# seemapoudel58/Physics_informed_image_segmentation

Hardware: AMD Instinct MI355X
Metric: training images/sec (512x512, Stage-II RD+PF loss) (higher is better)
Workload: dtype fp32 (fp16x3 split MFMA, power-of-two block scales; direct + Winograd convs); 1 GPU; C2: UNet(1,1,64) bs=8/GPU 512x512 Stage-II (lambda_RD=lambda_PF=1e-4, D=5, a=0.5, eps=0.05) AdamW lr=1e-5; global_batch=8, parallelism=dp1

## Files before the change

### include/pis_capi.h

```cpp
#ifndef PIS_CAPI_H
#define PIS_CAPI_H

#include <stddef.h>
#include <stdint.h>

#ifdef __cplusplus
extern "C" {
#endif

typedef void* pis_stream_t;

#define PIS_OK 0
#define PIS_ERR_ARG (-1)
#define PIS_ERR_LAUNCH (-2)
#define PIS_ERR_WORKSPACE (-3)

#define PIS_RELU 1
#define PIS_SCALE 2
#define PIS_MASK 4
#define PIS_ACCUMULATE 8
#define PIS_WINO_PREPARED 16
#define PIS_W_UNFLIPPED 32
#define PIS_FILTER_READY 64

const char* pis_last_error(void);
int pis_version(void);

#define PIS_TUNE_IGEMM_BK 1
#define PIS_TUNE_DEBUG_NOLOAD 2
#define PIS_TUNE_CONV_HALO 3
#define PIS_TUNE_HALO_VARIANT 4
#define PIS_TUNE_WGRAD_VARIANT 5
#define PIS_TUNE_WGRAD_BLOCKS 6
#define PIS_TUNE_C1_WGRAD 7
#define PIS_TUNE_WINOGRAD 8
#define PIS_TUNE_WINO_WGRAD_BLOCKS 9
#define PIS_TUNE_WINO_TILE 10
#define PIS_TUNE_WINO_F4 11
#define PIS_TUNE_WINO_FUSED 12
#define PIS_TUNE_CONVT_GEMM 13
#define PIS_TUNE_WGRAD_X6 14
#define PIS_TUNE_WINO_GEMM_OUT 15
#define PIS_TUNE_WINO_DZ2 16
#define PIS_TUNE_WINO_VW 17
#define PIS_TUNE_LOSS_ROWS 18
#define PIS_TUNE_LOSS_ROWMUL 19
#define PIS_TUNE_SLAB_CHUNKS 20
#define PIS_TUNE_WGRAD_PAIR 21
#define PIS_TUNE_WINO_GEMM_OUT_H3 22
#define PIS_TUNE_WINO_H3_PRE 23
#define PIS_TUNE_WINO_PERSIST 24
#define PIS_TUNE_FUSED_STAGGER 25
#define PIS_TUNE_FUSED_WIDE 26
#define PIS_TUNE_FUSED_K128 27
#define PIS_TUNE_FUSED_PAIR 28
#define PIS_TUNE_DIRECT_H3 29
#define PIS_TUNE_DIRECT_WG 30
#define PIS_TUNE_WGRAD_T 31
#define PIS_TUNE_DIRECT_PIPE 32
#define PIS_TUNE_DIRECT_W8 33
#define PIS_TUNE_DIRECT_WSTRIP 34
#define PIS_TUNE_DIRECT_WBLOCKS 35
#define PIS_TUNE_HEAD_LOSS_ROWS 36
#define PIS_TUNE_DIRECT_WGRAD_ALL 37
#define PIS_TUNE_HEAD_LOSS_WIDE 38
#define PIS_TUNE_WGRAD_T_DEPTH 39
#define PIS_TUNE_DZ_VW 40
#define PIS_TUNE_GEMM_256 41
#define PIS_TUNE_LAST_WGRAD_MAIN 42
#define PIS_TUNE_DIRECT_W_VWALK 43
#define PIS_TUNE_DIRECT_WGRAD_MAIN 44
#define PIS_TUNE_GEMM_PRIO 45
#define PIS_TUNE_WINO_OUT_MPF 46
#define PIS_TUNE_WINO_F6 47
#define PIS_TUNE_WGRAD_OUT 48
#define PIS_TUNE_DIRECT_W_ROWS 49
#define PIS_TUNE_WINO_XFORM 50
#define PIS_TUNE_WINO_DGRAD_T 51
#define PIS_TUNE_PROB_VARIANT 52
#define PIS_TUNE_DIRECT_MFMA16 53
#define PIS_TUNE_EVOLVE_T 54
#define PIS_TUNE_EDT_PRUNE 55
#define PIS_TUNE_NKEYS 56
#define PIS_DEBUG_NOLOAD (1 << 16)
int pis_tune(int key, int value);
int pis_debug_gemm_nt(const float* A, const float* B, float* C, int M, int N, int K, int batch, int variant,
                      pis_stream_t stream);
int pis_debug_stream_probe(const float* a, const float* b, float* dst, int64_t n, float* partial, int grid,
                           pis_stream_t stream);

int pis_debug_band_probe(const float* a, int64_t n, int mode, float* partial, int grid, pis_stream_t stream);

int pis_arm_gemm_event(void* event);

int pis_stream_create(int priority, pis_stream_t* out);
int pis_stream_destroy(pis_stream_t stream);
int pis_stream_capture_status(pis_stream_t stream);

typedef void (*pis_launch_hook_t)(const char* kernel, int phase, pis_stream_t stream, double flop,
                                  void* user);
void pis_set_launch_hook(pis_launch_hook_t fn, void* user);

int pis_conv3x3_fwd(const float* x, int ldx, const float* w_krsc, const float* bias,
                    const float* scale, float* y, int ldy, int B, int H, int W, int Cin,
                    int Cout, int flags, pis_stream_t stream);
size_t pis_conv3x3_ex_ws(int B, int H, int W, int Cin, int Cout);
int pis_conv3x3_fwd_ex(const float* x, int ldx, const float* w_krsc, const float* bias,
                       const float* scale, float* y, int ldy, int B, int H, int W, int Cin, int Cout,
                       int flags, void* ws, size_t ws_bytes, pis_stream_t stream);
int pis_conv3x3_flip(const float* w_krsc, float* w_flip, int Cin, int Cout, pis_stream_t stream);
int pis_conv3x3_dgrad(const float* dz, int ldz, const float* w_flip, const float* mask, int ldm,
                      const float* scale, float* dx, int lddx, int B, int H, int W, int Cin,
                      int Cout, int flags, pis_stream_t stream);
int pis_conv3x3_dgrad_ex(const float* dz, int ldz, const float* w_flip, const float* mask, int ldm,
                         const float* scale, float* dx, int lddx, int B, int H, int W, int Cin,
                         int Cout, int flags, void* ws, size_t ws_bytes, pis_stream_t stream);
size_t pis_conv3x3_keep_bytes(int B, int H, int W, int Cin, int Cout);
int pis_conv3x3_fwd_keep(const float* x, int ldx, const float* w_krsc, const float* bias,
                         const float* scale, float* y, int ldy, int B, int H, int W, int Cin, int Cout,
                         int flags, void* ws, size_t ws_bytes, float* keep, pis_stream_t stream);
int pis_conv3x3_fwd_pool(const float* x, int ldx, const float* w_krsc, const float* bias, const float* scale,
                         float* y, int ldy, int B, int H, int W, int Cin, int Cout, int flags, void* ws,
                         size_t ws_bytes, float* keep, float* pool, pis_stream_t stream);
int pis_conv3x3_wgrad_keep(const float* x, int ldx, const float* dz, int ldz, float* dw_krsc, float* db,
                           int B, int H, int W, int Cin, int Cout, int flags, void* ws, size_t ws_bytes,
                           const float* keep, pis_stream_t stream);
size_t pis_conv3x3_filter_bytes(int B, int H, int W, int Cin, int Cout, int dgrad);
int pis_conv3x3_filter(const float* w, int B, int H, int W, int Cin, int Cout, int dgrad, void* out,
                       size_t out_bytes, pis_stream_t stream);
typedef struct pis_filter_job {
  const float* w;
  void* out;
  size_t out_bytes;
  int B, H, W, Cin, Cout, dgrad;
} pis_filter_job;
#define PIS_FILTER_MAX_JOBS 40
int pis_conv3x3_filter_format(int B, int H, int W, int Cin, int Cout, int dgrad);
int pis_conv3x3_filters(const pis_filter_job* jobs, int n, pis_stream_t stream);
int pis_conv3x3_dgrad_direct(int B, int H, int W, int Cin, int Cout, int ldz, size_t ws_bytes);
int pis_conv3x3_bwd_prep(const float* dz, int ldz, int B, int H, int W, int Cin, int Cout, void* ws_dgrad,
                         size_t ws_dgrad_bytes, void* ws_wgrad, size_t ws_wgrad_bytes, pis_stream_t stream);
size_t pis_conv3x3_wgrad_ws(int B, int H, int W, int Cin, int Cout);
int pis_conv3x3_wgrad(const float* x, int ldx, const float* dz, int ldz, float* dw_krsc, float* db,
                      int B, int H, int W, int Cin, int Cout, int flags, void* ws, size_t ws_bytes,
                      pis_stream_t stream);

int pis_convt2x2_fwd(const float* x, int ldx, const float* w_ijoc, const float* bias, float* y,
                     int ldy, int B, int H, int W, int Cin, int Cout, pis_stream_t stream);
int pis_convt2x2_prep(const float* w_ijoc, float* w_cijo, int Cin, int Cout, pis_stream_t stream);
int pis_convt2x2_dgrad(const float* dy, int lddy, const float* w_cijo, const float* mask, int ldm,
                       float* dx, int lddx, int B, int H, int W, int Cin, int Cout, int flags,
                       pis_stream_t stream);
size_t pis_convt2x2_wgrad_ws(int B, int H, int W, int Cin, int Cout);
int pis_convt2x2_wgrad(const float* x, int ldx, const float* dy, int lddy, float* dw_ijoc,
                       float* db, int B, int H, int W, int Cin, int Cout, int flags, void* ws,
                       size_t ws_bytes, pis_stream_t stream);

int pis_maxpool2x2_fwd(const float* x, int ldx, float* y, int B, int H, int W, int C,
                       pis_stream_t stream);
int pis_maxpool2x2_bwd(const float* x, int ldx, const float* dy, const float* dskip, int ldskip,
                       float* dx, int lddx, int B, int H, int W, int C, pis_stream_t stream);

int pis_head_fwd(const float* x, int ldx, const float* w, const float* b, float* z, float* u,
                 int64_t npix, int C, pis_stream_t stream);
size_t pis_head_bwd_ws(int64_t npix, int C);
int pis_head_bwd(const float* x, int ldx, const float* w, const float* g, const float* u, float* dx,
                 int lddx, float* dw, float* db, int64_t npix, int C, int flags, void* ws,
                 size_t ws_bytes, pis_stream_t stream);

typedef struct pis_loss_params {
  float dice_w, bce_w;
  float rd_w, pf_w;
  float smooth;
  float D, a;
  float eps;
  float thr;
  int flags;
} pis_loss_params;
#define PIS_LOSS_ALL_TERMS 1
#define PIS_LOSS_CHAIN_SIGMOID 2
#define PIS_LOSS_NO_REACTION 4
#define PIS_LOSS_NTERMS 8
size_t pis_loss_ws(int B, int H, int W);
int pis_loss_fwd(const float* p, const float* t, int B, int H, int W, const pis_loss_params* prm,
                 float* out_terms, int* counts, float* scores, void* ws, size_t ws_bytes,
                 pis_stream_t stream);
int pis_loss_bwd(const float* p, const float* t, int B, int H, int W, const pis_loss_params* prm,
                 const float* terms, const float* grad_out, float* dst, int flags,
                 pis_stream_t stream);

size_t pis_head_loss_fwd_ws(int B, int H, int W);
int pis_head_loss_fwd_ok(int B, int H, int W, int C);
int pis_head_loss_fwd(const float* x, int ldx, const float* w, const float* bias, const float* t, float* z,
                      float* u, int B, int H, int W, int C, const pis_loss_params* prm, float* out_terms,
                      int* counts, float* scores, void* ws, size_t ws_bytes, pis_stream_t stream);
size_t pis_head_loss_bwd_ws(int B, int H, int W, int C);
int pis_head_loss_bwd(const float* x, int ldx, const float* w, const float* u, const float* t,
                      float* du_out, int B, int H, int W, int C, const pis_loss_params* prm,
                      const float* terms, const float* grad_out, float* dx, int lddx, float* dw,
                      float* db, int flags, void* ws, size_t ws_bytes, pis_stream_t stream);
int pis_pde_fields(const float* u, int B, int H, int W, float D, float a, float* lap,
                   float* residual, float* gradmag2, pis_stream_t stream);
int pis_pde_fields_bwd(const float* u, const float* g_lap, const float* g_residual,
                       const float* g_gradmag2, int B, int H, int W, float D, float a, float* du,
                       pis_stream_t stream);

int pis_adamw_step(float* p, const float* g, float* m, float* v, int64_t n, double lr, double beta1,
                   double beta2, double eps, double weight_decay, double step_size, double bc2_sqrt,
                   double grad_scale, pis_stream_t stream);

#define PIS_GRADNORM_SKIP_NONFINITE 1
#define PIS_GRADNORM_NSTATS 8
size_t pis_grad_sumsq_ws(int n_seg, int64_t n_total);
int pis_grad_sumsq(const float* g, const int64_t* seg_off, const int64_t* seg_len, int n_seg,
                   double grad_scale, double max_norm ,
                   int flags , double* seg_sumsq, void* record,
                   void* stats, void* ws, size_t ws_bytes, pis_stream_t stream);
int pis_adamw_step_clipped(float* p, const float* g, float* m, float* v, int64_t n, double lr,
                           double beta1, double beta2, double eps, double weight_decay,
                           double step_size, double bc2_sqrt, double grad_scale, const void* record,
                           pis_stream_t stream);

int pis_adamw_step_ema(float* p, const float* g, float* m, float* v, float* ema, int64_t n, double lr,
                       double beta1, double beta2, double eps, double weight_decay, double step_size,
                       double bc2_sqrt, double grad_scale, double ema_weight,
                       const void* record , pis_stream_t stream);
int pis_arena_exchange(float* a, float* b, int64_t n, pis_stream_t stream);

size_t pis_colsum_ws(int64_t npix, int C);
int pis_colsum(const float* src, int ld, int64_t npix, int C, float* out, int flags, void* ws,
               size_t ws_bytes, pis_stream_t stream);

size_t pis_synth_ws(int B, int H, int W);
int pis_synth_discs(const float* discs, const int* ndisc, int max_discs, uint64_t seed,
                    const int64_t* sample_ids, float* img, float* mask, int B, int H, int W,
                    void* ws, size_t ws_bytes, pis_stream_t stream);

size_t pis_boundary_ws(int B, int H, int W);
int pis_boundary_metrics(const float* p, const float* t, int B, int H, int W, float thr, int tolerance,
// ... 58 lines not shown
```

### physics_informed_image_segmentation_amd/_hip.py

```python
from __future__ import annotations

import ctypes
import os
from ctypes import c_double, c_float, c_int, c_int64, c_size_t, c_void_p
from typing import Optional

import torch

_HERE = os.path.dirname(os.path.abspath(__file__))
LIB_PATH = os.path.join(_HERE, "_lib", "libpis.so")

PIS_RELU, PIS_SCALE, PIS_MASK, PIS_ACCUMULATE, PIS_WINO_PREPARED, PIS_W_UNFLIPPED = 1, 2, 4, 8, 16, 32
PIS_FILTER_READY = 64
PIS_LOSS_ALL_TERMS, PIS_LOSS_CHAIN_SIGMOID, PIS_LOSS_NO_REACTION = 1, 2, 4
PIS_TUNE_LAST_WGRAD_MAIN = 42
PIS_TUNE_DIRECT_MFMA16 = 53
PIS_TUNE_PROB_VARIANT = 52
PIS_TUNE_EVOLVE_T = 54
PIS_TUNE_EDT_PRUNE = 55
PIS_EVOLVE_CLAMP, PIS_EVOLVE_TILE_H, PIS_EVOLVE_TILE_W, PIS_EVOLVE_MAX_STEPS = 1, 32, 64, 65536
PIS_CACHE_IMG_U8, PIS_CACHE_IMG_F32, PIS_CACHE_MASK_BITS, PIS_CACHE_MASK_F32 = 0, 1, 0, 1
PIS_GRADNORM_SKIP_NONFINITE, PIS_GRADNORM_NSTATS = 1, 8
LOSS_NTERMS = 8
TERM_TOTAL, TERM_DICE, TERM_BCE, TERM_RD, TERM_PF, TERM_I, TERM_P, TERM_T = range(8)


class FilterJob(ctypes.Structure):
    _fields_ = [("w", c_void_p), ("out", c_void_p), ("out_bytes", c_size_t), ("B", c_int), ("H", c_int),
                ("W", c_int), ("Cin", c_int), ("Cout", c_int), ("dgrad", c_int)]


class LossParams(ctypes.Structure):
    _fields_ = [("dice_w", c_float), ("bce_w", c_float), ("rd_w", c_float), ("pf_w", c_float),
                ("smooth", c_float), ("D", c_float), ("a", c_float), ("eps", c_float),
                ("thr", c_float), ("flags", c_int)]


P, I, L, Z, Dbl = c_void_p, c_int, c_int64, c_size_t, c_double
LAUNCH_HOOK_T = ctypes.CFUNCTYPE(None, ctypes.c_char_p, c_int, c_void_p, ctypes.c_double, c_void_p)

_SIGNATURES = {
    "pis_set_launch_hook": ([LAUNCH_HOOK_T, P], None),
    "pis_arm_gemm_event": ([P], c_int),
    "pis_stream_create": ([I, ctypes.POINTER(c_void_p)], c_int),
    "pis_stream_destroy": ([P], c_int),
    "pis_stream_capture_status": ([P], c_int),
    "pis_version": ([], c_int),
    "pis_last_error": ([], ctypes.c_char_p),
    "pis_tune": ([I, I], c_int),
    "pis_debug_gemm_nt": ([P, P, P, I, I, I, I, I, P], c_int),
    "pis_debug_stream_probe": ([P, P, P, L, P, I, P], c_int),
    "pis_debug_band_probe": ([P, L, I, P, I, P], c_int),
    "pis_conv3x3_dgrad_direct": ([I, I, I, I, I, I, Z], c_int),
    "pis_conv3x3_bwd_prep": ([P, I, I, I, I, I, I, P, Z, P, Z, P], c_int),
    "pis_conv3x3_filter_bytes": ([I, I, I, I, I, I], c_size_t),
    "pis_conv3x3_filter_format": ([I, I, I, I, I, I], c_int),
    "pis_conv3x3_filter": ([P, I, I, I, I, I, I, P, Z, P], c_int),
    "pis_conv3x3_filters": ([P, I, P], c_int),
    "pis_conv3x3_fwd_pool": ([P, I, P, P, P, P, I, I, I, I, I, I, I, P, Z, P, P, P], c_int),
    "pis_conv3x3_fwd": ([P, I, P, P, P, P, I, I, I, I, I, I, I, P], c_int),
    "pis_conv3x3_flip": ([P, P, I, I, P], c_int),
    "pis_conv3x3_dgrad": ([P, I, P, P, I, P, P, I, I, I, I, I, I, I, P], c_int),
    "pis_conv3x3_ex_ws": ([I, I, I, I, I], c_size_t),
    "pis_conv3x3_fwd_ex": ([P, I, P, P, P, P, I, I, I, I, I, I, I, P, Z, P], c_int),
    "pis_conv3x3_dgrad_ex": ([P, I, P, P, I, P, P, I, I, I, I, I, I, I, P, Z, P], c_int),
    "pis_conv3x3_wgrad_ws": ([I, I, I, I, I], c_size_t),
    "pis_conv3x3_keep_bytes": ([I, I, I, I, I], c_size_t),
    "pis_conv3x3_fwd_keep": ([P, I, P, P, P, P, I, I, I, I, I, I, I, P, Z, P, P], c_int),
    "pis_conv3x3_wgrad_keep": ([P, I, P, I, P, P, I, I, I, I, I, I, P, Z, P, P], c_int),
    "pis_conv3x3_wgrad": ([P, I, P, I, P, P, I, I, I, I, I, I, P, Z, P], c_int),
    "pis_convt2x2_fwd": ([P, I, P, P, P, I, I, I, I, I, I, P], c_int),
    "pis_convt2x2_prep": ([P, P, I, I, P], c_int),
    "pis_convt2x2_dgrad": ([P, I, P, P, I, P, I, I, I, I, I, I, I, P], c_int),
    "pis_convt2x2_wgrad_ws": ([I, I, I, I, I], c_size_t),
    "pis_convt2x2_wgrad": ([P, I, P, I, P, P, I, I, I, I, I, I, P, Z, P], c_int),
    "pis_maxpool2x2_fwd": ([P, I, P, I, I, I, I, P], c_int),
    "pis_maxpool2x2_bwd": ([P, I, P, P, I, P, I, I, I, I, I, P], c_int),
    "pis_head_fwd": ([P, I, P, P, P, P, L, I, P], c_int),
    "pis_head_bwd_ws": ([L, I], c_size_t),
    "pis_head_bwd": ([P, I, P, P, P, P, I, P, P, L, I, I, P, Z, P], c_int),
    "pis_loss_ws": ([I, I, I], c_size_t),
    "pis_loss_fwd": ([P, P, I, I, I, ctypes.POINTER(LossParams), P, P, P, P, Z, P], c_int),
    "pis_loss_bwd": ([P, P, I, I, I, ctypes.POINTER(LossParams), P, P, P, I, P], c_int),
    "pis_head_loss_fwd_ws": ([I, I, I], c_size_t),
    "pis_head_loss_fwd_ok": ([I, I, I, I], c_int),
    "pis_head_loss_fwd": ([P, I, P, P, P, P, P, I, I, I, I, ctypes.POINTER(LossParams), P, P, P, P, Z, P], c_int),
    "pis_head_loss_bwd_ws": ([I, I, I, I], c_size_t),
    "pis_head_loss_bwd": ([P, I, P, P, P, P, I, I, I, I, ctypes.POINTER(LossParams), P, P, P, I, P, P, I, P, Z,
                           P], c_int),
    "pis_adamw_step": ([P, P, P, P, L, Dbl, Dbl, Dbl, Dbl, Dbl, Dbl, Dbl, Dbl, P], c_int),
    "pis_grad_sumsq_ws": ([I, L], c_size_t),
    "pis_grad_sumsq": ([P, P, P, I, Dbl, Dbl, I, P, P, P, P, Z, P], c_int),
    "pis_adamw_step_clipped": ([P, P, P, P, L, Dbl, Dbl, Dbl, Dbl, Dbl, Dbl, Dbl, Dbl, P, P], c_int),
    "pis_adamw_step_ema": ([P, P, P, P, P, L, Dbl, Dbl, Dbl, Dbl, Dbl, Dbl, Dbl, Dbl, Dbl, P, P], c_int),
    "pis_arena_exchange": ([P, P, L, P], c_int),
    "pis_colsum_ws": ([L, I], c_size_t),
    "pis_colsum": ([P, I, L, I, P, I, P, Z, P], c_int),
    "pis_pde_fields": ([P, I, I, I, c_float, c_float, P, P, P, P], c_int),
    "pis_pde_fields_bwd": ([P, P, P, P, I, I, I, c_float, c_float, P, P], c_int),
    "pis_synth_ws": ([I, I, I], c_size_t),
    "pis_synth_discs": ([P, P, I, ctypes.c_uint64, P, P, P, I, I, I, P, Z, P], c_int),
    "pis_boundary_ws": ([I, I, I], c_size_t),
    "pis_boundary_metrics": ([P, P, I, I, I, c_float, I, P, P, P, P, Z, P], c_int),
    "pis_objects_ws": ([I, I, I], c_size_t),
    "pis_object_metrics": ([P, P, I, I, I, c_float, I, I, P, P, P, P, Z, P], c_int),
    "pis_probability_ws": ([I, I, I], c_size_t),
    "pis_probability_table": ([P, P, I, I, I, P, P, P, Z, P], c_int),
    "pis_cache_batch": ([P, I, Z, P, I, Z, P, P, P, L, P, P, I, I, I, P], c_int),
    "pis_cache_batch_affine": ([P, I, Z, P, I, Z, P, P, P, L, P, P, I, I, I, P], c_int),
    "pis_tile_count": ([I, I, I, I, I, ctypes.POINTER(c_int), ctypes.POINTER(c_int)], c_int),
    "pis_tile_gather": ([P, I, Z, P, I, I, I, I, I, I, I, L, L, P, P], c_int),
    "pis_tile_blend": ([P, I, I, I, I, I, I, I, c_float, P, P, P], c_int),
    "pis_pde_evolve_ws": ([I, I, I, I], c_size_t),
    "pis_pde_evolve": ([P, P, P, P, I, I, I, c_float, c_float, c_float, c_float, c_float, I, I, c_float, P, Z, P],
                       c_int),
    "pis_pde_energies_ws": ([I, I, I], c_size_t),
    "pis_pde_energies": ([P, I, I, I, c_float, c_float, c_float, P, P, P, Z, P], c_int),
    "pis_edt_ws": ([I, I, I], c_size_t),
    "pis_edt_sq": ([P, I, I, I, P, P, Z, P], c_int),
    "pis_surface_distances_ws": ([I, I, I], c_size_t),
    "pis_surface_distances": ([P, P, I, I, I, P, P, P, Z, P], c_int),
}

_lib: Optional[ctypes.CDLL] = None


class HipError(RuntimeError):
    pass


def lib() -> ctypes.CDLL:
    global _lib
    if _lib is None:
        if not os.path.exists(LIB_PATH):
            raise HipError(f"HIP extension not built: {LIB_PATH} is missing "
                           "(run __graft_entry__.build() or `python -m physics_informed_image_segmentation_amd.build`)")
        import torch
        so = ctypes.CDLL(LIB_PATH)
        for name, (argtypes, restype) in _SIGNATURES.items():
            fn = getattr(so, name)
            fn.argtypes = argtypes
            fn.restype = restype
        _lib = so
    return _lib


def exported_symbols():
    return list(_SIGNATURES)


def ptr(t: Optional[torch.Tensor]) -> int:
    return 0 if t is None else t.data_ptr()


def stream_handle(device: Optional[torch.device] = None) -> int:
    return torch.cuda.current_stream(device).cuda_stream


# ... 108 lines not shown
```

### physics_informed_image_segmentation_amd/csrc/capi.hip

```cpp
#include <atomic>
#include <cstdarg>

#include "common.h"

namespace pis {
static thread_local char g_last_error[512] = "";

void set_error(const char* fmt, ...) {
  va_list ap;
  va_start(ap, fmt);
  vsnprintf(g_last_error, sizeof(g_last_error), fmt, ap);
  va_end(ap);
}

static std::atomic<int> g_tune[PIS_TUNE_NKEYS] = {0, 16, 0, 1, 0, 1, 512, 0, 1, 1024, 4, 1, 0, 4, 3, 1, 1, 2,
                                                   1, 1, 1, 0, 1, 0, 0, 0, 2, 1, 0, 1, 0, 1, 1, 0, 0, 512, 0, 0, 1, 2, 2, 0, 1, 1, 0, 0, 1,
                                                   0, 1, 2, 1, 1, 0, 3, 8, 3};

int tune_get(int key) { return (key > 0 && key < PIS_TUNE_NKEYS) ? g_tune[key].load() : 0; }

static std::atomic<pis_launch_hook_t> g_hook{nullptr};
static std::atomic<void*> g_hook_user{nullptr};

void launch_hook(const char* kernel, int phase, hipStream_t s, double flop) {
  const pis_launch_hook_t fn = g_hook.load(std::memory_order_relaxed);
  if (fn) fn(kernel, phase, (pis_stream_t)s, flop, g_hook_user.load(std::memory_order_relaxed));
}

static thread_local hipEvent_t g_gemm_event = nullptr;

void gemm_done(hipStream_t s) {
  if (g_gemm_event) {
    (void)hipEventRecord(g_gemm_event, s);
    g_gemm_event = nullptr;
  }
}
}

extern "C" const char* pis_last_error(void) { return pis::g_last_error; }
extern "C" int pis_version(void) { return 1; }

extern "C" int pis_arm_gemm_event(void* event) {
  const int pending = pis::g_gemm_event != nullptr;
  pis::g_gemm_event = (hipEvent_t)event;
  return pending;
}

extern "C" int pis_stream_create(int priority, pis_stream_t* out) {
  PIS_CHECK_ARG(out != nullptr, "pis_stream_create: out is NULL");
  hipStream_t s = nullptr;
  const hipError_t e = hipStreamCreateWithPriority(&s, hipStreamNonBlocking, priority);
  if (e != hipSuccess) {
    pis::set_error("pis_stream_create: %s", hipGetErrorString(e));
    return PIS_ERR_LAUNCH;
  }
  *out = (pis_stream_t)s;
  return PIS_OK;
}

extern "C" int pis_stream_destroy(pis_stream_t stream) {
  PIS_CHECK_ARG(stream != nullptr, "pis_stream_destroy: NULL stream");
  const hipError_t e = hipStreamDestroy((hipStream_t)stream);
  if (e != hipSuccess) {
    pis::set_error("pis_stream_destroy: %s", hipGetErrorString(e));
    return PIS_ERR_LAUNCH;
  }
  return PIS_OK;
}

extern "C" int pis_stream_capture_status(pis_stream_t stream) {
  hipStreamCaptureStatus st = hipStreamCaptureStatusNone;
  const hipError_t e = hipStreamIsCapturing((hipStream_t)stream, &st);
  if (e != hipSuccess) {
    pis::set_error("pis_stream_capture_status: %s", hipGetErrorString(e));
    return PIS_ERR_LAUNCH;
  }
  return (int)st;
}

extern "C" void pis_set_launch_hook(pis_launch_hook_t fn, void* user) {
  pis::g_hook_user.store(user);
  pis::g_hook.store(fn);
}

extern "C" int pis_tune(int key, int value) {
  if (key <= 0 || key >= PIS_TUNE_NKEYS) {
    pis::set_error("pis_tune: unknown key %d", key);
    return PIS_ERR_ARG;
  }
  if (key == PIS_TUNE_IGEMM_BK && value >= 0 && value != 16 && value != 32) {
    pis::set_error("pis_tune: igemm K-step must be 16 or 32");
    return PIS_ERR_ARG;
  }
  if (key == PIS_TUNE_EVOLVE_T && value >= 0 && value != 1 && value != 2 && value != 4 && value != 8) {
    pis::set_error("pis_tune: the temporal block of pis_pde_evolve must be 1, 2, 4 or 8");
    return PIS_ERR_ARG;
  }
  if (key == PIS_TUNE_EDT_PRUNE && value >= 0 && value != 0 && value != 1 && value != 3) {
    pis::set_error("pis_tune: the pruning of the distance transform's row pass must be 0, 1 or 3");
    return PIS_ERR_ARG;
// ... 6 lines not shown
```

### physics_informed_image_segmentation_amd/csrc/wgrad.hip

```cpp
#include "conv3x3_plan.h"

namespace pis {

enum BMode { B_PLAIN = 0, B_CONV3 = 1, B_CONV3_C1 = 2 };

struct WgradArgs {
  const float* a; int lda; int a_up2; int Ca;
  const float* b; int ldb; int b_mode; int Cb;
  int B, H, W;
  int P;
  int Mp, Np;
  int pix_per_split;
  float* part;
  float* part_bias;
  int64_t bs_a, bs_b, bs_part, split_stride;
  int pair;
  int bias_xi;
  int dbg;
};

template <int BM, int BN, int BKP>
__global__ __launch_bounds__(256) void wgrad_f32_kernel(WgradArgs g) {
  const Remap2 rm = xcd_remap2();
  if (rm.batch) {
// ... 1049 lines not shown
#pragma unroll
          for (int a = 0; a < 2; ++a)
#pragma unroll
            for (int b = 0; b < 2; ++b) acc[a][b] = (acc[a][b] * fa) * fb;
        }
        ua = sa;
        ub = sb;
      }
    }
#pragma unroll
    for (int ks = 0; ks < 2; ++ks) {
      if (ks) {
#pragma unroll
        for (int pl = 0; pl < 2; ++pl)
#pragma unroll
          for (int a = 0; a < 2; ++a) {
            af[pl][a] = frag(buf + pl * WT_PLANE, 1, 64 * wm + 32 * a);
            bf[pl][a] = frag(buf + (2 + pl) * WT_PLANE, 1, 64 * wn + 32 * a);
          }
      }
#pragma unroll
      for (int a = 0; a < 2; ++a)
#pragma unroll
        for (int b = 0; b < 2; ++b) {
          acc[a][b] = __builtin_amdgcn_mfma_f32_32x32x16_f16(af[1][a], bf[0][b], acc[a][b], 0, 0, 0);
          acc[a][b] = __builtin_amdgcn_mfma_f32_32x32x16_f16(af[0][a], bf[1][b], acc[a][b], 0, 0, 0);
          acc[a][b] = __builtin_amdgcn_mfma_f32_32x32x16_f16(af[0][a], bf[0][b], acc[a][b], 0, 0, 0);
        }
    }
  };
  using I0 = std::integral_constant<int, 0>;
  using I1 = std::integral_constant<int, 1>;
  using I2 = std::integral_constant<int, 2>;
  if constexpr (D == 2) {
#pragma unroll 1
    for (int st = 0; st < nst; st += 2) {
      kstep(st, I0{}, I0{});
      if (st + 1 < nst) kstep(st + 1, I1{}, I1{});
    }
  } else {
#pragma unroll 1
    for (int st = 0; st < nst; st += 6) {
      kstep(st, I0{}, I0{});
      if (st + 1 < nst) kstep(st + 1, I1{}, I1{});
      if (st + 2 < nst) kstep(st + 2, I0{}, I2{});
      if (st + 3 < nst) kstep(st + 3, I1{}, I0{});
      if (st + 4 < nst) kstep(st + 4, I0{}, I1{});
      if (st + 5 < nst) kstep(st + 5, I1{}, I2{});
    }
  }
  float* out = g.part + (size_t)split * (g.split_stride ? g.split_stride : (int64_t)g.Mp * g.Np);
  const float inv_a = ua != 0.f ? 1.f / ua : 0.f, inv_b = ub != 0.f ? 1.f / ub : 0.f;
  if (TW && (g.dbg & 4)) {
    float t = 0.f;
#pragma unroll
    for (int a = 0; a < 2; ++a)
#pragma unroll
      for (int b = 0; b < 2; ++b)
#pragma unroll
        for (int r = 0; r < 16; ++r) t += acc[a][b][r];
    if (t == 1.2345f) out[tid] = t;
    return;
  }
#pragma unroll
  for (int a = 0; a < 2; ++a)
#pragma unroll
    for (int b = 0; b < 2; ++b) {
      const int n = n0 + 64 * wn + 32 * b + li;
#pragma unroll
      for (int r = 0; r < 16; ++r) {
        const int m = m0 + 64 * wm + 32 * a + (r & 3) + 8 * (r >> 2) + 4 * lh;
        out[(size_t)m * g.Np + n] = (acc[a][b][r] * inv_a) * inv_b;
      }
    }
  if (do_bias) {
    __syncthreads();
    f32x4* rb4 = reinterpret_cast<f32x4*>(smem);
    rb4[tid] = bsum;
    __syncthreads();
    if (tid < 32) {
      f32x4 t = rb4[tid];
#pragma unroll
      for (int r = 1; r < 8; ++r) t += rb4[32 * r + tid];
      *reinterpret_cast<f32x4*>(g.part_bias + (size_t)split * g.Mp + m0 + 4 * tid) = t;
    }
  }
}

static bool h3t_exact(const WgradArgs& a) {
  return a.P % WT_BK == 0 && a.pix_per_split % WT_BK == 0 &&
         ((int64_t)a.P + WT_BK) * std::max(a.a_up2 ? 0 : a.lda, a.ldb) * 4 < (int64_t(1) << 31);
}

static int run_wgrad(const WgradArgs& base, const WgradPlan& pl, hipStream_t s, int batches = 1) {
  WgradArgs a = base;
  a.pix_per_split = pl.pps;
  a.pair = tune_get(PIS_TUNE_WGRAD_PAIR);
  a.dbg = tune_get(PIS_TUNE_DEBUG_NOLOAD);
  const int tiles = (a.Mp / pl.bm) * (a.Np / pl.bn);
  const dim3 grid(tiles * pl.splits, batches);
  const int x6 = tune_get(PIS_TUNE_WGRAD_X6);
  const bool plain = a.b_mode == B_PLAIN;
  const int cin = plain ? a.Np : a.Cb;
  if ((x6 == 2 || (x6 == 3 && cin >= 256)) && plain && pl.pps % 16 == 0 &&
      (!a.a_up2 || a.W % 8 == 0)) {
    if (tune_get(PIS_TUNE_WGRAD_T) != 0 && pl.bm == 128 && pl.bn == 128 && !a.a_up2 &&
        pl.pps % WT_BK == 0 && a.lda % 4 == 0 && a.ldb % 4 == 0 && a.bs_a % 4 == 0 && a.bs_b % 4 == 0 &&
        ((uintptr_t)a.a & 15) == 0 && ((uintptr_t)a.b & 15) == 0) {
      if (a.dbg)
        hipLaunchKernelGGL((wgrad_h3t_kernel<false, 2, true>), grid, dim3(256), 0, s, a);
      else if (h3t_exact(a))
        hipLaunchKernelGGL((wgrad_h3t_kernel<false, 2, false, true>), grid, dim3(256), 0, s, a);
      else
        hipLaunchKernelGGL((wgrad_h3t_kernel<false, 2>), grid, dim3(256), 0, s, a);
      return launch_status("wgrad_h3t");
    }
    if (pl.bm == 128 && pl.bn == 128) hipLaunchKernelGGL((wgrad_h3_kernel<128, 128>), grid, dim3(256), 0, s, a);
    else if (pl.bm == 128) hipLaunchKernelGGL((wgrad_h3_kernel<128, 64>), grid, dim3(256), 0, s, a);
    else if (pl.bn == 128) hipLaunchKernelGGL((wgrad_h3_kernel<64, 128>), grid, dim3(256), 0, s, a);
    else hipLaunchKernelGGL((wgrad_h3_kernel<64, 64>), grid, dim3(256), 0, s, a);
    return launch_status("wgrad_h3");
  }
  if (x6 != 0 && a.b_mode == B_PLAIN && pl.pps % 16 == 0 && (!a.a_up2 || a.W % 8 == 0)) {
    if (pl.bm == 128 && pl.bn == 128) hipLaunchKernelGGL((wgrad_x6_kernel<128, 128>), grid, dim3(256), 0, s, a);
    else if (pl.bm == 128) hipLaunchKernelGGL((wgrad_x6_kernel<128, 64>), grid, dim3(256), 0, s, a);
    else if (pl.bn == 128) hipLaunchKernelGGL((wgrad_x6_kernel<64, 128>), grid, dim3(256), 0, s, a);
    else hipLaunchKernelGGL((wgrad_x6_kernel<64, 64>), grid, dim3(256), 0, s, a);
    return launch_status("wgrad_x6");
  }
  if (pl.bm == 128 && pl.bn == 128)
    hipLaunchKernelGGL((wgrad_f32_kernel<128, 128, 16>), grid, dim3(256), 0, s, a);
  else if (pl.bm == 128)
    hipLaunchKernelGGL((wgrad_f32_kernel<128, 64, 32>), grid, dim3(256), 0, s, a);
  else if (pl.bn == 128)
    hipLaunchKernelGGL((wgrad_f32_kernel<64, 128, 32>), grid, dim3(256), 0, s, a);
  else
    hipLaunchKernelGGL((wgrad_f32_kernel<64, 64, 32>), grid, dim3(256), 0, s, a);
  return launch_status("wgrad_f32");
}

}

using namespace pis;

extern "C" size_t pis_colsum_ws(int64_t npix, int C) { return colsum_ws(npix, C); }

extern "C" int pis_colsum(const float* src, int ld, int64_t npix, int C, float* out, int flags,
                          void* ws, size_t ws_bytes, pis_stream_t stream) {
  PIS_CHECK_ARG(src && out && npix > 0 && C > 0, "pis_colsum: bad arguments");
  PIS_CHECK_ARG(C % 4 != 0 || ld % 4 == 0, "pis_colsum: ld must be a multiple of 4");
  PIS_CHECK_ARG(ld >= C, "pis_colsum: ld must be at least C");
  PIS_CHECK_ARG(ws && ws_bytes >= colsum_ws(npix, C), "pis_colsum: workspace missing or too small");
  PIS_CHECK_ARG(C % 4 != 0 || ((uintptr_t)src | (uintptr_t)ws) % 16 == 0,
                "pis_colsum: src and ws must be 16-byte aligned when C is a multiple of 4");
  return colsum(src, ld, npix, C, out, flags & PIS_ACCUMULATE, ws, ws_bytes, (hipStream_t)stream);
}

__global__ __launch_bounds__(256) void wgrad_c1_kernel(const float* __restrict__ x, int ldx,
                                                       const float* __restrict__ dz, int ldz, int B, int H,
                                                       int W, int Cout, int64_t pix_per_block,
                                                       float* __restrict__ part, float* __restrict__ part_b) {
  __shared__ f32x4 red[256][10];
  const int lanes = Cout / 4, groups = 256 / lanes;
  const int lp = threadIdx.x / lanes, q = threadIdx.x - lp * lanes, c4 = 4 * q;
  f32x4 acc[10];
#pragma unroll
// ... 185 lines not shown
  PIS_CHECK_ARG((Cin == 1 || ldx % 4 == 0) && ldz % 4 == 0, "pis_conv3x3_wgrad: ld must be multiples of 4");
  hipStream_t s = (hipStream_t)stream;
  const int acc = flags & PIS_ACCUMULATE;
  const WgradAlgo algo = resolve_wgrad(p, x, dz, ws_bytes);
  if (algo == WGRAD_NONE) return PIS_ERR_ARG;
  if (algo == WGRAD_DIRECT)
    return launch_direct_wgrad(x, ldx, dz, ldz, dw_krsc, db, B, H, W, Cin, Cout, acc, ws, ws_bytes, s);
  if (algo == WGRAD_WINO4 || algo == WGRAD_WINO2)
    return wino_wgrad(x, ldx, dz, ldz, dw_krsc, db, B, H, W, Cin, Cout, acc, p.wino_w, ws, s);
  if (algo == WGRAD_HALO) {
    const HaloPlan& hp = p.halo_w;
    W3Args a{};
    a.x = x; a.ldx = ldx; a.dz = dz; a.ldz = ldz;
    a.B = B; a.H = H; a.W = W; a.Cin = Cin; a.Cout = Cout;
    a.seg_per_split = hp.seg_per_split; a.nseg = hp.nseg;
    a.part = (float*)ws;
    a.part_bias = db ? (float*)((char*)ws + cdiv(hp.part_bytes, 256) * 256) : nullptr;
    const int tiles = (Cout / 64) * (Cin / 64);
    const double flop = 2.0 * (double)B * H * W * Cout * 9.0 * Cin;
    launch_hook("wgrad3x3_halo", 0, s, flop);
    if (tune_get(PIS_TUNE_WGRAD_VARIANT) != 0)
      hipLaunchKernelGGL((wgrad3x3_halo_kernel<2>), dim3(tiles * hp.splits), dim3(256), 0, s, a);
    else
      hipLaunchKernelGGL((wgrad3x3_halo_kernel<1>), dim3(tiles * hp.splits), dim3(256), 0, s, a);
    launch_hook("wgrad3x3_halo", 1, s, flop);
    int rc = launch_status("wgrad3x3_halo");
    if (!rc) rc = reduce_slabs2(a.part, hp.splits, (int64_t)Cout * 9 * Cin, dw_krsc, a.part_bias, hp.splits, Cout, db,
                                acc, s);
    return rc;
  }
  if (algo == WGRAD_C1_STREAM) {
    PIS_CHECK_ARG(Cout <= 1024 && Cout % 4 == 0, "pis_conv3x3_wgrad: Cin == 1 needs Cout % 4 == 0, <= 1024");
    const int64_t npix = (int64_t)B * H * W;
    const int64_t ppb = cdiv(npix, C1_BLOCKS);
    const int blocks = (int)cdiv(npix, ppb);
    float* part = (float*)ws;
    float* part_b = db ? part + (size_t)C1_BLOCKS * 9 * Cout : nullptr;
    const bool row = Cout == 64 && W % 64 == 0 && ldz % 4 == 0;
    if (row && H % 4 == 0)
      hipLaunchKernelGGL(wgrad_c1_row_kernel<4>, dim3(C1_BLOCKS), dim3(256), 0, s, x, ldx, dz, ldz, B, H, W, part,
                         part_b);
    else if (row)
      hipLaunchKernelGGL(wgrad_c1_row_kernel<1>, dim3(C1_BLOCKS), dim3(256), 0, s, x, ldx, dz, ldz, B, H, W, part,
                         part_b);
    else
      hipLaunchKernelGGL(wgrad_c1_kernel, dim3(blocks), dim3(256), 0, s, x, ldx, dz, ldz, B, H, W, Cout, ppb,
                         part, part_b);
    int rc = launch_status("wgrad_c1");
    const int nslab = row ? C1_BLOCKS : blocks;
    if (!rc) rc = reduce_slabs2(part, nslab, (int64_t)9 * Cout, dw_krsc, db ? part_b : nullptr, nslab, Cout, db, acc, s);
    return rc;
  }
  const WgradPlan& pl = p.gemm_w;
  WgradArgs a{};
  a.a = dz; a.lda = ldz; a.a_up2 = 0; a.Ca = Cout;
  a.b = x; a.ldb = ldx; a.b_mode = Cin == 1 ? B_CONV3_C1 : B_CONV3; a.Cb = Cin;
  a.B = B; a.H = H; a.W = W; a.P = B * H * W; a.Mp = Cout; a.Np = Cin == 1 ? 64 : 9 * Cin;
  a.part = (float*)ws;
  a.part_bias = db ? bias_slabs(ws, pl) : nullptr;
  int rc = run_wgrad(a, pl, s);
  if (rc) return rc;
  if (Cin == 1) {
    float* full = (float*)((char*)ws + wgrad_ws_bytes(pl));
    rc = reduce_slabs(a.part, pl.splits, (int64_t)Cout * 64, full, 0, s);
    if (!rc) {
      hipLaunchKernelGGL(compact_c1_kernel, dim3((unsigned)cdiv(Cout * 9, 256)), dim3(256), 0, s, full,
                         dw_krsc, Cout, acc);
      rc = launch_status("compact_c1");
    }
  } else {
    return reduce_slabs2(a.part, pl.splits, (int64_t)a.Mp * a.Np, dw_krsc, a.part_bias, pl.splits, Cout, db, acc, s);
  }
  if (rc || !db) return rc;
  return reduce_slabs(a.part_bias, pl.splits, Cout, db, acc, s);
}

static bool convt_wgrad_t_ok(int B, int H, int W, int Cin, int Cout, int ldx, int lddy, const void* x,
                             const void* dy) {
  return tune_get(PIS_TUNE_CONVT_GEMM) == 4 && W % 32 == 0 && (4 * Cout) % 128 == 0 && Cin >= 256 && Cin % 128 == 0 &&
         ldx % 4 == 0 && lddy % 4 == 0 && ((uintptr_t)x & 15) == 0 && ((uintptr_t)dy & 15) == 0 &&
         plan_wgrad(4 * Cout, Cin, B * H * W, 4 * Cout, Cin).pps % WT_BK == 0;
}

extern "C" size_t pis_convt2x2_wgrad_ws(int B, int H, int W, int Cin, int Cout) {
  return std::max(wgrad_ws_bytes(plan_wgrad(4 * Cout, Cin, B * H * W, Cout, Cin)),
                  wgrad_ws_bytes(plan_wgrad(4 * Cout, Cin, B * H * W, 4 * Cout, Cin)));
}

extern "C" int pis_convt2x2_wgrad(const float* x, int ldx, const float* dy, int lddy, float* dw_ijoc,
                                  float* db, int B, int H, int W, int Cin, int Cout, int flags,
                                  void* ws, size_t ws_bytes, pis_stream_t stream) {
  PIS_CHECK_ARG(x && dy && dw_ijoc && B > 0 && H > 0 && W > 0 && Cin > 0 && Cout > 0,
                "pis_convt2x2_wgrad: bad arguments");
  PIS_CHECK_ARG(Cin % 64 == 0 && Cout % 64 == 0, "pis_convt2x2_wgrad: Cin/Cout must be multiples of 64");
  PIS_CHECK_ARG(ldx % 4 == 0 && lddy % 4 == 0, "pis_convt2x2_wgrad: ld must be multiples of 4");
  PIS_CHECK_ARG(ws && ws_bytes >= pis_convt2x2_wgrad_ws(B, H, W, Cin, Cout),
                "pis_convt2x2_wgrad: workspace too small");
  hipStream_t s = (hipStream_t)stream;
  const int acc = flags & PIS_ACCUMULATE;
  const int P = B * H * W;
  if (convt_wgrad_t_ok(B, H, W, Cin, Cout, ldx, lddy, x, dy)) {
    const WgradPlan pl = plan_wgrad(4 * Cout, Cin, P, 4 * Cout, Cin);
    WgradArgs a{};
    a.a = dy; a.lda = lddy; a.a_up2 = 1; a.Ca = Cout;
    a.b = x; a.ldb = ldx; a.b_mode = B_PLAIN; a.Cb = Cin;
    a.B = B; a.H = H; a.W = W; a.P = P; a.Mp = 4 * Cout; a.Np = Cin; a.part = (float*)ws;
    a.part_bias = db ? bias_slabs(ws, pl) : nullptr;
    a.pix_per_split = pl.pps;
    const int tiles = (a.Mp / 128) * (a.Np / 128);
    if (h3t_exact(a))
      hipLaunchKernelGGL((wgrad_h3t_kernel<true, 2, false, true>), dim3(tiles * pl.splits), dim3(256), 0, s, a);
    else
      hipLaunchKernelGGL((wgrad_h3t_kernel<true, 2>), dim3(tiles * pl.splits), dim3(256), 0, s, a);
    int rc = launch_status("wgrad_h3t<up2>");
    if (!rc) rc = reduce_slabs2(a.part, pl.splits, (int64_t)a.Mp * a.Np, dw_ijoc, a.part_bias, pl.splits * 4, Cout, db,
                                acc, s);
    return rc;
  }
  const WgradPlan pl = plan_wgrad(4 * Cout, Cin, P, Cout, Cin);
  WgradArgs a{};
  a.a = dy; a.lda = lddy; a.a_up2 = 1; a.Ca = Cout;
  a.b = x; a.ldb = ldx; a.b_mode = B_PLAIN; a.Cb = Cin;
  a.B = B; a.H = H; a.W = W; a.P = P; a.Mp = 4 * Cout; a.Np = Cin; a.part = (float*)ws;
  a.part_bias = db ? bias_slabs(ws, pl) : nullptr;
  int rc = run_wgrad(a, pl, s);
  if (!rc) rc = reduce_slabs2(a.part, pl.splits, (int64_t)a.Mp * a.Np, dw_ijoc, a.part_bias, pl.splits * 4, Cout, db,
                              acc, s);
  return rc;
}
```

Baseline: 391.1 images/s.

## Add 256x128 tiled up2 wgrad kernel for transposed-conv weight gradients

```diff
diff --git a/include/pis_capi.h b/include/pis_capi.h
--- a/include/pis_capi.h
+++ b/include/pis_capi.h
@@ -81,7 +81,8 @@
 #define PIS_TUNE_DIRECT_MFMA16 53
 #define PIS_TUNE_EVOLVE_T 54
 #define PIS_TUNE_EDT_PRUNE 55
-#define PIS_TUNE_NKEYS 56
+#define PIS_TUNE_CONVT_WGRAD_TILE 56
+#define PIS_TUNE_NKEYS 57
 #define PIS_DEBUG_NOLOAD (1 << 16)
 int pis_tune(int key, int value);
 int pis_debug_gemm_nt(const float* A, const float* B, float* C, int M, int N, int K, int batch, int variant,
@@ -155,6 +156,7 @@
 int pis_convt2x2_wgrad(const float* x, int ldx, const float* dy, int lddy, float* dw_ijoc,
                        float* db, int B, int H, int W, int Cin, int Cout, int flags, void* ws,
                        size_t ws_bytes, pis_stream_t stream);
+int pis_debug_convt2x2_wgrad_tile_splits(int B, int H, int W, int Cin, int Cout);
 
 int pis_maxpool2x2_fwd(const float* x, int ldx, float* y, int B, int H, int W, int C,
                        pis_stream_t stream);
diff --git a/physics_informed_image_segmentation_amd/_hip.py b/physics_informed_image_segmentation_amd/_hip.py
--- a/physics_informed_image_segmentation_amd/_hip.py
+++ b/physics_informed_image_segmentation_amd/_hip.py
@@ -18,6 +18,7 @@
 PIS_TUNE_PROB_VARIANT = 52
 PIS_TUNE_EVOLVE_T = 54
 PIS_TUNE_EDT_PRUNE = 55
+PIS_TUNE_CONVT_WGRAD_TILE = 56
 PIS_EVOLVE_CLAMP, PIS_EVOLVE_TILE_H, PIS_EVOLVE_TILE_W, PIS_EVOLVE_MAX_STEPS = 1, 32, 64, 65536
 PIS_CACHE_IMG_U8, PIS_CACHE_IMG_F32, PIS_CACHE_MASK_BITS, PIS_CACHE_MASK_F32 = 0, 1, 0, 1
 PIS_GRADNORM_SKIP_NONFINITE, PIS_GRADNORM_NSTATS = 1, 8
@@ -74,6 +75,7 @@
     "pis_convt2x2_dgrad": ([P, I, P, P, I, P, I, I, I, I, I, I, I, P], c_int),
     "pis_convt2x2_wgrad_ws": ([I, I, I, I, I], c_size_t),
     "pis_convt2x2_wgrad": ([P, I, P, I, P, P, I, I, I, I, I, I, P, Z, P], c_int),
+    "pis_debug_convt2x2_wgrad_tile_splits": ([I, I, I, I, I], c_int),
     "pis_maxpool2x2_fwd": ([P, I, P, I, I, I, I, P], c_int),
     "pis_maxpool2x2_bwd": ([P, I, P, P, I, P, I, I, I, I, I, P], c_int),
     "pis_head_fwd": ([P, I, P, P, P, P, L, I, P], c_int),
diff --git a/physics_informed_image_segmentation_amd/csrc/capi.hip b/physics_informed_image_segmentation_amd/csrc/capi.hip
--- a/physics_informed_image_segmentation_amd/csrc/capi.hip
+++ b/physics_informed_image_segmentation_amd/csrc/capi.hip
@@ -15,7 +15,7 @@
 
 static std::atomic<int> g_tune[PIS_TUNE_NKEYS] = {0, 16, 0, 1, 0, 1, 512, 0, 1, 1024, 4, 1, 0, 4, 3, 1, 1, 2,
                                                    1, 1, 1, 0, 1, 0, 0, 0, 2, 1, 0, 1, 0, 1, 1, 0, 0, 512, 0, 0, 1, 2, 2, 0, 1, 1, 0, 0, 1,
-                                                   0, 1, 2, 1, 1, 0, 3, 8, 3};
+                                                   0, 1, 2, 1, 1, 0, 3, 8, 3, 1};
 
 int tune_get(int key) { return (key > 0 && key < PIS_TUNE_NKEYS) ? g_tune[key].load() : 0; }
 
diff --git a/physics_informed_image_segmentation_amd/csrc/wgrad.hip b/physics_informed_image_segmentation_amd/csrc/wgrad.hip
--- a/physics_informed_image_segmentation_amd/csrc/wgrad.hip
+++ b/physics_informed_image_segmentation_amd/csrc/wgrad.hip
@@ -1155,6 +1155,184 @@
       f32x4 t = rb4[tid];
 #pragma unroll
       for (int r = 1; r < 8; ++r) t += rb4[32 * r + tid];
+      *reinterpret_cast<f32x4*>(g.part_bias + (size_t)split * g.Mp + m0 + 4 * tid) = t;
+    }
+  }
+}
+
+constexpr int WU_BM = 256, WU_BN = 128;
+constexpr int WU_LDS = 6 * WT_PLANE;
+
+__global__ __launch_bounds__(256, 2) void wgrad_up2_tile_kernel(WgradArgs g) {
+  __shared__ __attribute__((aligned(16))) _Float16 smem[WU_LDS];
+  __shared__ float red[2][2][4];
+  const int tid = threadIdx.x, lane = tid & 63, wave = tid >> 6;
+  const int wm = wave & 1, wn = wave >> 1, li = lane & 31, lh = lane >> 5;
+  const int ntn = g.Np / WU_BN;
+  const int tiles = (g.Mp / WU_BM) * ntn;
+  const int bid = xcd_remap(blockIdx.x, gridDim.x);
+  const int split = bid / tiles;
+  const int tile = bid - split * tiles;
+  const int m0 = (tile / ntn) * WU_BM, n0 = (tile % ntn) * WU_BN;
+  const int p_begin = split * g.pix_per_split;
+  const int p_end = min(g.P, p_begin + g.pix_per_split);
+  const int nst = max(0, (p_end - p_begin) / WT_BK);
+  const int srow = tid >> 5, sc4 = tid & 31;
+  const float* gb = g.b + n0 + 4 * sc4;
+  const float* ga[2];
+#pragma unroll
+  for (int h = 0; h < 2; ++h) {
+    const int col = m0 + 128 * h + 4 * sc4, ij = col / g.Ca;
+    ga[h] = g.a + (col - ij * g.Ca) + ((size_t)(ij >> 1) * (2 * g.W) + (ij & 1)) * g.lda;
+  }
+  const bool do_bias = g.part_bias != nullptr && n0 == 0;
+  f32x4 bsum[2] = {{0.f, 0.f, 0.f, 0.f}, {0.f, 0.f, 0.f, 0.f}};
+
+  f32x4 xa[2][4], xb[4];
+  auto gload = [&](int st) __attribute__((always_inline)) {
+    const int p0 = p_begin + st * WT_BK;
+    const int hw = g.H * g.W, b = p0 / hw, rem = p0 - b * hw, y = rem / g.W, x0 = rem - y * g.W;
+    const size_t abase = (((size_t)b * 2 * g.H + 2 * y) * (2 * g.W) + 2 * x0) * g.lda;
+#pragma unroll
+    for (int j = 0; j < 4; ++j) {
+      const int r = srow + 8 * j;
+#pragma unroll
+      for (int h = 0; h < 2; ++h) xa[h][j] = *reinterpret_cast<const f32x4*>(ga[h] + abase + (size_t)(2 * r) * g.lda);
+      xb[j] = *reinterpret_cast<const f32x4*>(gb + (size_t)(p0 + r) * g.ldb);
+    }
+  };
+  auto publish = [&](int par) __attribute__((always_inline)) {
+    if (do_bias) {
+#pragma unroll
+      for (int j = 0; j < 4; ++j) {
+        bsum[0] += xa[0][j];
+        bsum[1] += xa[1][j];
+      }
+    }
+    const float ma = wave_max_nonneg(absmax_x4(xa));
+    const float mb = wave_max_nonneg(absmax_x4(xb));
+    if (lane == 0) {
+      red[par][0][wave] = ma;
+      red[par][1][wave] = mb;
+    }
+  };
+  float sa = 0.f, sb = 0.f, sa_min = __builtin_inff(), sb_min = __builtin_inff();
+  auto split_store = [&](int par) __attribute__((always_inline)) {
+    auto umax4 = [](const float (&r)[4]) __attribute__((always_inline)) {
+      return __uint_as_float(max(max(__float_as_uint(r[0]), __float_as_uint(r[1])),
+                                 max(__float_as_uint(r[2]), __float_as_uint(r[3]))));
+    };
+    sa = h3_keep(sa, umax4(red[par][0]), sa_min);
+    sb = h3_keep(sb, umax4(red[par][1]), sb_min);
+#pragma unroll
+    for (int j = 0; j < 4; ++j) {
+      const int off = wtsw(srow + 8 * j, sc4 >> 1) + 4 * (sc4 & 1);
+      u32x2 h, l;
+#pragma unroll
+      for (int hf = 0; hf < 2; ++hf) {
+        split2h_x4(xa[hf][j] * sa, h, l);
+        *reinterpret_cast<u32x2*>(smem + hf * WT_PLANE + off) = h;
+        *reinterpret_cast<u32x2*>(smem + (2 + hf) * WT_PLANE + off) = l;
+      }
+      split2h_x4(xb[j] * sb, h, l);
+      *reinterpret_cast<u32x2*>(smem + 4 * WT_PLANE + off) = h;
+      *reinterpret_cast<u32x2*>(smem + 5 * WT_PLANE + off) = l;
+    }
+  };
+
+  const int gq = lane >> 4, q = (lane & 15) >> 2, pp = lane & 3;
+  const int kh = gq >> 1, chk = 2 * (gq & 1) + (pp >> 1), slot = 4 * (pp & 1);
+  auto frag = [&](const _Float16* plane, int ks, int col0) __attribute__((always_inline)) {
+    const int row = 16 * ks + 8 * kh + q, ch = col0 / 8 + chk;
+    const s16x4 lo4 = tr_read(plane + wtsw(row, ch) + slot);
+    const s16x4 hi4 = tr_read(plane + wtsw(row + 4, ch) + slot);
+    return __builtin_bit_cast(f16x8, __builtin_shufflevector(lo4, hi4, 0, 1, 2, 3, 4, 5, 6, 7));
+  };
+  const _Float16* a_hi = smem + wm * WT_PLANE;
+  const _Float16* a_lo = smem + (2 + wm) * WT_PLANE;
+  const _Float16* b_hi = smem + 4 * WT_PLANE;
+  const _Float16* b_lo = smem + 5 * WT_PLANE;
+
+  f32x16 acc[4][2];
+#pragma unroll
+  for (int a = 0; a < 4; ++a)
+#pragma unroll
+    for (int b = 0; b < 2; ++b)
+#pragma unroll
+      for (int r = 0; r < 16; ++r) acc[a][b][r] = 0.f;
+  float ua = 0.f, ub = 0.f;
+
+  if (nst > 0) {
+    gload(0);
+    publish(0);
+    __syncthreads();
+    split_store(0);
+    if (nst > 1) gload(1);
+  }
+#pragma unroll 1
+  for (int st = 0; st < nst; ++st) {
+    __syncthreads();
+    if (sa != ua || sb != ub) {
+      if (ua != 0.f) {
+        const float fa = sa / ua, fb = sb / ub;
+#pragma unroll
+        for (int a = 0; a < 4; ++a)
+#pragma unroll
+          for (int b = 0; b < 2; ++b) acc[a][b] = (acc[a][b] * fa) * fb;
+      }
+      ua = sa;
+      ub = sb;
+    }
+#pragma unroll
+    for (int ks = 0; ks < 2; ++ks) {
+      f16x8 bf[2][2];
+#pragma unroll
+      for (int b = 0; b < 2; ++b) {
+        bf[0][b] = frag(b_hi, ks, 64 * wn + 32 * b);
+        bf[1][b] = frag(b_lo, ks, 64 * wn + 32 * b);
+      }
+#pragma unroll
+      for (int a = 0; a < 4; ++a) {
+        const f16x8 ah = frag(a_hi, ks, 32 * a), al = frag(a_lo, ks, 32 * a);
+#pragma unroll
+        for (int b = 0; b < 2; ++b) {
+          acc[a][b] = __builtin_amdgcn_mfma_f32_32x32x16_f16(al, bf[0][b], acc[a][b], 0, 0, 0);
+          acc[a][b] = __builtin_amdgcn_mfma_f32_32x32x16_f16(ah, bf[1][b], acc[a][b], 0, 0, 0);
+          acc[a][b] = __builtin_amdgcn_mfma_f32_32x32x16_f16(ah, bf[0][b], acc[a][b], 0, 0, 0);
+        }
+      }
+    }
+    const bool more = st + 1 < nst;
+    if (more) publish((st + 1) & 1);
+    __syncthreads();
+    if (more) {
+      split_store((st + 1) & 1);
+      if (st + 2 < nst) gload(st + 2);
+    }
+  }
+  float* out = g.part + (size_t)split * g.Mp * g.Np;
+  const float inv_a = ua != 0.f ? 1.f / ua : 0.f, inv_b = ub != 0.f ? 1.f / ub : 0.f;
+#pragma unroll
+  for (int a = 0; a < 4; ++a)
+#pragma unroll
+    for (int b = 0; b < 2; ++b) {
+      const int n = n0 + 64 * wn + 32 * b + li;
+#pragma unroll
+      for (int r = 0; r < 16; ++r) {
+        const int m = m0 + 128 * wm + 32 * a + (r & 3) + 8 * (r >> 2) + 4 * lh;
+        out[(size_t)m * g.Np + n] = (acc[a][b][r] * inv_a) * inv_b;
+      }
+    }
+  if (do_bias) {
+    f32x4* rb4 = reinterpret_cast<f32x4*>(smem);
+    rb4[tid] = bsum[0];
+    rb4[256 + tid] = bsum[1];
+    __syncthreads();
+    if (tid < 64) {
+      const int base = 256 * (tid >> 5) + (tid & 31);
+      f32x4 t = rb4[base];
+#pragma unroll
+      for (int r = 1; r < 8; ++r) t += rb4[base + 32 * r];
       *reinterpret_cast<f32x4*>(g.part_bias + (size_t)split * g.Mp + m0 + 4 * tid) = t;
     }
   }
@@ -1506,9 +1684,41 @@
          plan_wgrad(4 * Cout, Cin, B * H * W, 4 * Cout, Cin).pps % WT_BK == 0;
 }
 
+static bool convt_wgrad_tile_shape(int W, int Cin, int Cout) {
+  return W % WT_BK == 0 && Cin % WU_BN == 0 && (4 * Cout) % WU_BM == 0;
+}
+
+static WgradPlan plan_convt_tile(int Mp, int Np, int P) {
+  WgradPlan p{};
+  p.bm = WU_BM;
+  p.bn = WU_BN;
+  const int tiles = (Mp / WU_BM) * (Np / WU_BN);
+  const int64_t want_splits = std::max<int64_t>(1, cdiv(512, tiles));
+  int64_t pps = std::min<int64_t>(std::max<int64_t>(512, cdiv(P, want_splits)), 8192);
+  pps = cdiv(pps, WT_BK) * WT_BK;
+  p.pps = (int)pps;
+  p.splits = (int)cdiv(P, pps);
+  p.part_bytes = (size_t)p.splits * Mp * Np * sizeof(float);
+  p.bias_bytes = (size_t)p.splits * Mp * sizeof(float);
+  return p;
+}
+
+static bool convt_wgrad_tile_ok(int W, int Cin, int Cout, int ldx, int lddy, const void* x, const void* dy) {
+  return tune_get(PIS_TUNE_CONVT_WGRAD_TILE) != 0 && tune_get(PIS_TUNE_CONVT_GEMM) == 4 &&
+         convt_wgrad_tile_shape(W, Cin, Cout) && ldx % 4 == 0 && lddy % 4 == 0 && ((uintptr_t)x & 15) == 0 &&
+         ((uintptr_t)dy & 15) == 0;
+}
+
 extern "C" size_t pis_convt2x2_wgrad_ws(int B, int H, int W, int Cin, int Cout) {
-  return std::max(wgrad_ws_bytes(plan_wgrad(4 * Cout, Cin, B * H * W, Cout, Cin)),
-                  wgrad_ws_bytes(plan_wgrad(4 * Cout, Cin, B * H * W, 4 * Cout, Cin)));
+  size_t n = std::max(wgrad_ws_bytes(plan_wgrad(4 * Cout, Cin, B * H * W, Cout, Cin)),
+                      wgrad_ws_bytes(plan_wgrad(4 * Cout, Cin, B * H * W, 4 * Cout, Cin)));
+  if (convt_wgrad_tile_shape(W, Cin, Cout)) n = std::max(n, wgrad_ws_bytes(plan_convt_tile(4 * Cout, Cin, B * H * W)));
+  return n;
+}
+
+extern "C" int pis_debug_convt2x2_wgrad_tile_splits(int B, int H, int W, int Cin, int Cout) {
+  if (B <= 0 || H <= 0 || W <= 0 || Cin <= 0 || Cout <= 0 || !convt_wgrad_tile_shape(W, Cin, Cout)) return 0;
+  return plan_convt_tile(4 * Cout, Cin, B * H * W).splits;
 }
 
 extern "C" int pis_convt2x2_wgrad(const float* x, int ldx, const float* dy, int lddy, float* dw_ijoc,
@@ -1523,6 +1733,21 @@
   hipStream_t s = (hipStream_t)stream;
   const int acc = flags & PIS_ACCUMULATE;
   const int P = B * H * W;
+  if (convt_wgrad_tile_ok(W, Cin, Cout, ldx, lddy, x, dy)) {
+    const WgradPlan pl = plan_convt_tile(4 * Cout, Cin, P);
+    WgradArgs a{};
+    a.a = dy; a.lda = lddy; a.a_up2 = 1; a.Ca = Cout;
+    a.b = x; a.ldb = ldx; a.b_mode = B_PLAIN; a.Cb = Cin;
+    a.B = B; a.H = H; a.W = W; a.P = P; a.Mp = 4 * Cout; a.Np = Cin; a.part = (float*)ws;
+    a.part_bias = db ? bias_slabs(ws, pl) : nullptr;
+    a.pix_per_split = pl.pps;
+    const int tiles = (a.Mp / WU_BM) * (a.Np / WU_BN);
+    hipLaunchKernelGGL(wgrad_up2_tile_kernel, dim3(tiles * pl.splits), dim3(256), 0, s, a);
+    int rc = launch_status("wgrad_up2_tile");
+    if (!rc) rc = reduce_slabs2(a.part, pl.splits, (int64_t)a.Mp * a.Np, dw_ijoc, a.part_bias, pl.splits * 4, Cout, db,
+                                acc, s);
+    return rc;
+  }
   if (convt_wgrad_t_ok(B, H, W, Cin, Cout, ldx, lddy, x, dy)) {
     const WgradPlan pl = plan_wgrad(4 * Cout, Cin, P, 4 * Cout, Cin);
     WgradArgs a{};
```

Measured after the change: 396.6 images/s (median of 6 runs). 1.4% higher.
